# Anttwo/MACARONS

Measured on AMD Instinct MI355X. Metric: candidate-camera coverage-gain evals/sec (100k pts, 200 cams), higher is better.
Workload: dtype f32; 1 GPU; scorer: B=1 cloud x N=100000 points x C=200 cameras per GPU (BASELINE headline 100k pts / 200 cams), inputs resident in HBM; points=100000, cams_per_gpu=200, parallelism=camera-shard x1, streams=2

## Files before the change

macarons_amd/csrc/local_pct6.hip:

```cpp
#include "lp_split.h"

namespace mcr {
namespace v6 {

typedef float f32x4 __attribute__((ext_vector_type(4)));

__device__ __forceinline__ int opaque(int v) {
    asm volatile("" : "+v"(v));
    return v;
}

constexpr int PF = 3;
struct WRing { uint4 b[PF][2]; };

__device__ __forceinline__ const uint4* wptr(const float* Wp, int nt, int S, int lane) {
    return reinterpret_cast<const uint4*>(Wp) + (size_t)nt * S * 2 * 64 + lane;
}
template <int S>
__device__ __forceinline__ void wload(WRing& r, const uint4* bp) {
#pragma unroll
    for (int p = 0; p < (S < PF ? S : PF); ++p) {
        r.b[p][0] = bp[(p * 2 + 0) * 64];
        r.b[p][1] = bp[(p * 2 + 1) * 64];
    }
    __builtin_amdgcn_sched_barrier(0);
}

__device__ __forceinline__ void pin(f32x16& a, f32x16& b) { asm volatile("" : "+v"(a), "+v"(b)); }
__device__ __forceinline__ void pin(f32x16& a, f32x16& b, f32x16& c) { asm volatile("" : "+v"(a), "+v"(b), "+v"(c)); }

__device__ __forceinline__ void zero(f32x16& a) {
#pragma unroll
    for (int r = 0; r < 16; ++r) a[r] = 0.f;
}

template <int S>
__device__ __forceinline__ void gemm(f32x16 (&acc)[2], const uint4* __restrict__ A, WRing& r, const uint4* __restrict__ bp,
                                     int lane_) {
    const int lane = opaque(lane_);
    const int i = lane & 31, h = lane >> 5, key = i & 15;
    Split2 an[2];
    auto fetch = [&](int s) {
        const int c = (2 * s + h) ^ key;
#pragma unroll
        for (int mt = 0; mt < 2; ++mt) {
            an[mt].hi = A[(0 * 64 + mt * 32 + i) * 16 + c];
            an[mt].lo = A[(1 * 64 + mt * 32 + i) * 16 + c];
        }
    };
    fetch(0);
#pragma unroll
    for (int s = 0; s < S; ++s) {
        const Split2 a0 = an[0], a1 = an[1];
        if (s + 1 < S) fetch(s + 1);
        const uint4 whi = r.b[s % PF][0], wlo = r.b[s % PF][1];
        if (s + PF < S) {
            r.b[s % PF][0] = bp[((s + PF) * 2 + 0) * 64];
            r.b[s % PF][1] = bp[((s + PF) * 2 + 1) * 64];
        }
        __builtin_amdgcn_sched_barrier(0);
        acc[0] = mfma_h(wlo, a0.hi, acc[0]);
        acc[1] = mfma_h(wlo, a1.hi, acc[1]);
        acc[0] = mfma_h(whi, a0.lo, acc[0]);
        acc[1] = mfma_h(whi, a1.lo, acc[1]);
        acc[0] = mfma_h(whi, a0.hi, acc[0]);
        acc[1] = mfma_h(whi, a1.hi, acc[1]);
        pin(acc[0], acc[1]);
        __builtin_amdgcn_sched_barrier(0);
    }
}

template <int S, class Fn>
__device__ __forceinline__ void gemm_with(f32x16 (&acc)[2], const uint4* __restrict__ A, WRing& r, const uint4* __restrict__ bp,
                                          int lane_, Fn fn) {
    const int lane = opaque(lane_);
    const int i = lane & 31, h = lane >> 5, key = i & 15;
    Split2 an[2];
    auto fetch = [&](int s) {
        const int c = (2 * s + h) ^ key;
#pragma unroll
        for (int mt = 0; mt < 2; ++mt) {
            an[mt].hi = A[(0 * 64 + mt * 32 + i) * 16 + c];
            an[mt].lo = A[(1 * 64 + mt * 32 + i) * 16 + c];
        }
    };
    fetch(0);
#pragma unroll
    for (int s = 0; s < S; ++s) {
        const Split2 a0 = an[0], a1 = an[1];
        if (s + 1 < S) fetch(s + 1);
        const uint4 whi = r.b[s % PF][0], wlo = r.b[s % PF][1];
        if (s + PF < S) {
            r.b[s % PF][0] = bp[((s + PF) * 2 + 0) * 64];
            r.b[s % PF][1] = bp[((s + PF) * 2 + 1) * 64];
        }
        __builtin_amdgcn_sched_barrier(0);
        acc[0] = mfma_h(wlo, a0.hi, acc[0]);
        acc[1] = mfma_h(wlo, a1.hi, acc[1]);
        acc[0] = mfma_h(whi, a0.lo, acc[0]);
        acc[1] = mfma_h(whi, a1.lo, acc[1]);
        acc[0] = mfma_h(whi, a0.hi, acc[0]);
        acc[1] = mfma_h(whi, a1.hi, acc[1]);
        fn(s);
        pin(acc[0], acc[1]);
        __builtin_amdgcn_sched_barrier(0);
    }
}

__device__ __forceinline__ void gemm_qkv(f32x16 (&acc)[2], f32x16& acch, const uint4* __restrict__ A, WRing& r0, WRing& r1,
                                         const uint4* __restrict__ bp0, const uint4* __restrict__ bp1, int wave, int lane_) {
    constexpr int S = 8;
    const int lane = opaque(lane_);
    const int i = lane & 31, h = lane >> 5, key = i & 15, mh = wave & 1;
    Split2 an[2];
    auto fetch = [&](int s) {
        const int c = (2 * s + h) ^ key;
#pragma unroll
        for (int mt = 0; mt < 2; ++mt) {
            an[mt].hi = A[(0 * 64 + mt * 32 + i) * 16 + c];
            an[mt].lo = A[(1 * 64 + mt * 32 + i) * 16 + c];
        }
    };
    fetch(0);
#pragma unroll
    for (int s = 0; s < S; ++s) {
        const Split2 a0 = an[0], a1 = an[1];
        const Split2 ah = mh ? a1 : a0;
        if (s + 1 < S) fetch(s + 1);
        const uint4 whi = r0.b[s % PF][0], wlo = r0.b[s % PF][1], vhi = r1.b[s % PF][0], vlo = r1.b[s % PF][1];
        if (s + PF < S) {
            r0.b[s % PF][0] = bp0[((s + PF) * 2 + 0) * 64];
            r0.b[s % PF][1] = bp0[((s + PF) * 2 + 1) * 64];
            r1.b[s % PF][0] = bp1[((s + PF) * 2 + 0) * 64];
            r1.b[s % PF][1] = bp1[((s + PF) * 2 + 1) * 64];
        }
        __builtin_amdgcn_sched_barrier(0);
        acc[0] = mfma_h(wlo, a0.hi, acc[0]);
        acc[1] = mfma_h(wlo, a1.hi, acc[1]);
        acch = mfma_h(vlo, ah.hi, acch);
        acc[0] = mfma_h(whi, a0.lo, acc[0]);
        acc[1] = mfma_h(whi, a1.lo, acc[1]);
        acch = mfma_h(vhi, ah.lo, acch);
        acc[0] = mfma_h(whi, a0.hi, acc[0]);
        acc[1] = mfma_h(whi, a1.hi, acc[1]);
        acch = mfma_h(vhi, ah.hi, acch);
        pin(acc[0], acc[1], acch);
        __builtin_amdgcn_sched_barrier(0);
    }
}

__device__ __forceinline__ void scale_add_bias(f32x16& x, float scale, const float* __restrict__ vec, int nt, int lane_) {
    const float4* p = reinterpret_cast<const float4*>(vec + 32 * nt + 4 * (opaque(lane_) >> 5));
#pragma unroll
    for (int g = 0; g < 4; ++g) {
        const float4 b = p[2 * g];
        x[4 * g] = fmaf(x[4 * g], scale, b.x); x[4 * g + 1] = fmaf(x[4 * g + 1], scale, b.y);
        x[4 * g + 2] = fmaf(x[4 * g + 2], scale, b.z); x[4 * g + 3] = fmaf(x[4 * g + 3], scale, b.w);
    }
}
__device__ __forceinline__ void init_bias(f32x16& a, const float* __restrict__ vec, int nt, int lane_) {
    const float4* p = reinterpret_cast<const float4*>(vec + 32 * nt + 4 * (opaque(lane_) >> 5));
#pragma unroll
    for (int g = 0; g < 4; ++g) {
        const float4 b = p[2 * g];
        a[4 * g] = b.x; a[4 * g + 1] = b.y; a[4 * g + 2] = b.z; a[4 * g + 3] = b.w;
    }
}

__device__ __forceinline__ void put4(uint2* __restrict__ planes, int idx, float v0, float v1, float v2, float v3) {
    uint2 hi, lo;
    split2h(v0, v1, hi.x, lo.x);
    split2h(v2, v3, hi.y, lo.y);
    planes[idx] = hi;
    planes[idx + 64 * 16 * 2] = lo;
}
template <class Fn>
__device__ __forceinline__ void put_planes(uint4* __restrict__ buf, int nt, int mt, const f32x16& t, int lane_, Fn f) {
    const int lane = opaque(lane_);
    const int j = lane & 31, h = lane >> 5, key = j & 15;
    uint2* b2 = reinterpret_cast<uint2*>(buf);
    const int base = (mt * 32 + j) * 32 + h;
#pragma unroll
    for (int g = 0; g < 4; ++g) {
        put4(b2, base + (((4 * nt + g) ^ key) << 1), f(t[4 * g], g, 0), f(t[4 * g + 1], g, 1), f(t[4 * g + 2], g, 2),
             f(t[4 * g + 3], g, 3));
        __builtin_amdgcn_sched_barrier(0);
    }
}
template <class Fn>
__device__ __forceinline__ void put_quad(uint4* __restrict__ buf, int nt, int mt, int g, const f32x16& t, int row, int key, Fn f) {
    uint2* b2 = reinterpret_cast<uint2*>(buf);
    put4(b2, mt * 1024 + row + (((4 * nt + g) ^ key) << 1), f(t[4 * g]), f(t[4 * g + 1]), f(t[4 * g + 2]), f(t[4 * g + 3]));
}
template <class Fn>
__device__ __forceinline__ void put_f32(float* __restrict__ buf, int LD, int chunk0, int mt, const f32x16& t, int lane_, Fn f) {
    const int lane = opaque(lane_);
    const int j = lane & 31, h = lane >> 5, key = j & 15;
    float* row = buf + (mt * 32 + j) * LD;
#pragma unroll
    for (int g = 0; g < 4; ++g)
        *reinterpret_cast<float4*>(row + (((chunk0 + 2 * g + h) ^ key) << 2)) =
            make_float4(f(t[4 * g], g, 0), f(t[4 * g + 1], g, 1), f(t[4 * g + 2], g, 2), f(t[4 * g + 3], g, 3));
}

__device__ __forceinline__ float halves_sum(float v) {
    const unsigned c = __builtin_bit_cast(unsigned, v);
    const auto q = __builtin_amdgcn_permlane32_swap(c, c, false, false);
    return __builtin_bit_cast(float, (unsigned)q[0]) + __builtin_bit_cast(float, (unsigned)q[1]);
}
template <class Op>
__device__ __forceinline__ float rows_allreduce(float v, Op op) {
    const unsigned b = __builtin_bit_cast(unsigned, v);
    const auto r = __builtin_amdgcn_permlane16_swap(b, b, false, false);
    v = op(__builtin_bit_cast(float, (unsigned)r[0]), __builtin_bit_cast(float, (unsigned)r[1]));
    const unsigned c = __builtin_bit_cast(unsigned, v);
    const auto q = __builtin_amdgcn_permlane32_swap(c, c, false, false);
    return op(__builtin_bit_cast(float, (unsigned)q[0]), __builtin_bit_cast(float, (unsigned)q[1]));
}

__device__ __forceinline__ void ln_partial(const f32x16 (&x)[2], float2* __restrict__ St, int wave, int lane_) {
    const int lane = opaque(lane_);
#pragma unroll
    for (int mt = 0; mt < 2; ++mt) {
        float s = 0.f;
#pragma unroll
        for (int r = 0; r < 16; r += 4) s += (x[mt][r] + x[mt][r + 1]) + (x[mt][r + 2] + x[mt][r + 3]);
        const float m = halves_sum(s) * (1.0f / 32.f);
        float q = 0.f;
#pragma unroll
        for (int r = 0; r < 16; ++r) {
            const float d = x[mt][r] - m;
            q = fmaf(d, d, q);
        }
        q = halves_sum(q);
        St[wave * 64 + mt * 32 + (lane & 31)] = make_float2(m, q);
    }
}
__device__ __forceinline__ void ln_finish(const f32x16 (&x)[2], const float2* __restrict__ St, uint4* __restrict__ P, int wave,
                                          int lane_) {
    const int j = opaque(lane_) & 31;
#pragma unroll
    for (int mt = 0; mt < 2; ++mt) {
        float2 p[4];
#pragma unroll
        for (int w = 0; w < 4; ++w) p[w] = St[w * 64 + mt * 32 + j];
        const float mu = ((p[0].x + p[1].x) + (p[2].x + p[3].x)) * 0.25f;
        float m2 = (p[0].y + p[1].y) + (p[2].y + p[3].y), dd = 0.f;
#pragma unroll
        for (int w = 0; w < 4; ++w) {
            const float d = p[w].x - mu;
            dd = fmaf(d, d, dd);
        }
        m2 = fmaf(32.f, dd, m2);
        const float rstd = 1.0f / sqrtf(m2 * (1.0f / 128.f) + 1e-5f);
        put_planes(P, wave, mt, x[mt], lane_, [&](float v, int, int) { return (v - mu) * rstd; });
    }
}

#ifdef L6_TRACE
__device__ long long l6_trace_buf[64];
#define L6_T() do { if (blockIdx.x == (L6_TRACE) && tid == 0) { l6_trace_buf[tp] = clock64(); l6_trace_buf[tp ? 63 : 62] = wall_clock64(); } ++tp; } while (0)
#else
#define L6_T() do { } while (0)
#endif

__global__ __launch_bounds__(256, 2) void local_pct6_kernel(const float* __restrict__ offs, float* __restrict__ feat,
                                                          long long ld_feat, long long S,
                                                          const float* __restrict__ blob, _Float16* __restrict__ feat_h,
                                                          _Float16* __restrict__ feat_l) {
    __shared__ __attribute__((aligned(16))) uint4 P[2 * 64 * 16];
    __shared__ __attribute__((aligned(16))) uint4 H[2 * 64 * 16];
    __shared__ __attribute__((aligned(16))) float2 St[4 * 64];
    float* Pq = reinterpret_cast<float*>(P);
    float* F = reinterpret_cast<float*>(H);
    const int tid = threadIdx.x, lane0 = tid & 63;
    const int wave = __builtin_amdgcn_readfirstlane(tid >> 6);
    const float* mats = blob;
    const float* vecs = blob + L6_MATS_TOTAL;
    const float* isc = vecs + L6_SCALES;
    const long long s0 = (long long)blockIdx.x * L3_QPB;
    const int lane = lane0;
    int tp = 0; (void)tp;
    L6_T();
    WRing ring;
    f32x16 acc[2], xres[2];
    wload<1>(ring, wptr(mats + l6_mat_off(0), wave, 1, lane));
    init_bias(acc[0], vecs + L3_VEC_EMB1, wave, lane);
    init_bias(acc[1], vecs + L3_VEC_EMB1, wave, lane);
    float xyz[2][3];
    {
        const int j = lane & 31;
#pragma unroll
        for (int mt = 0; mt < 2; ++mt) {
            const int t = mt * 32 + j;
            const long long seq = s0 + (t >> 4);
            xyz[mt][0] = xyz[mt][1] = xyz[mt][2] = 0.f;
            if (seq < S) {
                const float* p = offs + (seq * 16 + (t & 15)) * 3;
                xyz[mt][0] = p[0]; xyz[mt][1] = p[1]; xyz[mt][2] = p[2];
            }
        }
        const bool lowh = lane < 32;
#pragma unroll
        for (int mt = 0; mt < 2; ++mt) {
            Split2 a;
            a.hi = make_uint4(0, 0, 0, 0); a.lo = make_uint4(0, 0, 0, 0);
            split2h(lowh ? xyz[mt][0] : 0.f, lowh ? xyz[mt][1] : 0.f, a.hi.x, a.lo.x);
            split2h(lowh ? xyz[mt][2] : 0.f, 0.f, a.hi.y, a.lo.y);
            acc[mt] = mfma_h(ring.b[0][1], a.hi, acc[mt]);
            acc[mt] = mfma_h(ring.b[0][0], a.lo, acc[mt]);
            acc[mt] = mfma_h(ring.b[0][0], a.hi, acc[mt]);
        }
    }
    L6_T();
    wload<8>(ring, wptr(mats + l6_mat_off(1), wave, 8, lane));
    {
        const float sc = isc[0];
#pragma unroll
        for (int mt = 0; mt < 2; ++mt)
            put_planes(H, wave, mt, acc[mt], lane, [&](float v, int, int) { return l3_gelu(v * sc); });
    }
    init_bias(xres[0], vecs + L3_VEC_EMB2, wave, lane);
    init_bias(xres[1], vecs + L3_VEC_EMB2, wave, lane);
    __syncthreads();
    L6_T();
    gemm<8>(xres, H, ring, wptr(mats + l6_mat_off(1), wave, 8, lane), lane);
    L6_T();
    {
        const float sc = isc[1];
#pragma unroll
        for (int mt = 0; mt < 2; ++mt)
#pragma unroll
            for (int r = 0; r < 16; ++r) xres[mt][r] *= sc;
        const bool cat = wave == 3 && lane >= 32;
#pragma unroll
        for (int mt = 0; mt < 2; ++mt) {
            xres[mt][13] = cat ? xyz[mt][0] : xres[mt][13];
            xres[mt][14] = cat ? xyz[mt][1] : xres[mt][14];
            xres[mt][15] = cat ? xyz[mt][2] : xres[mt][15];
        }
    }

#pragma unroll 1
    for (int e = 0; e < 2; ++e) {
        const float* em = mats + l6_mat_off(2) + e * (L6_MAT_QKV + 5 * L6_MAT_128);
        const float* ev = vecs + L3_VEC_ENC0 + e * L3_VEC_ENC_STRIDE;
        const float* es = isc + 2 + 6 * e;
        const float* w_out = em + L6_MAT_QKV;
        const float* w_ff1a = w_out + L6_MAT_128;
        const float* w_ff1b = w_out + L6_MAT_128 * 2;
        const float* w_ff2a = w_out + L6_MAT_128 * 3;
        const float* w_ff2b = w_out + L6_MAT_128 * 4;
        WRing ring1;
        const uint4* bq0 = wptr(em, wave, 8, lane);
        const uint4* bq1 = wptr(em, 4 + (wave >> 1), 8, lane);
        wload<8>(ring, bq0);
        wload<8>(ring1, bq1);
        L6_T();
        ln_partial(xres, St, wave, lane);
        __syncthreads();
        L6_T();
        ln_finish(xres, St, P, wave, lane);
        __syncthreads();
        L6_T();
        {
            f32x16 aq[2], ah;
            const int nth = 4 + (wave >> 1);
            init_bias(aq[0], ev, wave, lane);
            init_bias(aq[1], ev, wave, lane);
            init_bias(ah, ev, nth, lane);
            gemm_qkv(aq, ah, P, ring, ring1, bq0, bq1, wave, lane);
            L6_T();
            wload<8>(ring, wptr(w_out, wave, 8, lane));
            const float sc = es[0];
            __syncthreads();
            L6_T();
            auto fb = [&](float v, int, int) { return v * sc; };
            float* dst = wave < 2 ? Pq : F;
            const int ld = wave < 2 ? 64 : 128, c0 = wave < 2 ? 8 * wave : 8 * (wave - 2);
#pragma unroll
            for (int mt = 0; mt < 2; ++mt) put_f32(dst, ld, c0, mt, aq[mt], lane, fb);
            put_f32(F, 128, 8 * (nth - 2), wave & 1, ah, lane, fb);
        }
        __syncthreads();
        L6_T();
        {
            const int ln = opaque(lane);
            const int r0 = wave * 16, li = ln & 15, g = ln >> 4;
            const int wq = ((r0 + li) * 64) | (li << 2) | g;
            const int wv = ((r0 + 4 * g) * 128) | ((((li >> 2) | (g << 2)) << 2)) | (li & 3);
            f32x4 pr[4];
#pragma unroll
            for (int hh = 0; hh < 4; ++hh) {
                f32x4 st = {0.f, 0.f, 0.f, 0.f};
#pragma unroll
                for (int sk = 0; sk < 2; ++sk) {
                    const float kk = Pq[wq ^ ((8 + 2 * hh + sk) << 2)];
                    const float qq = Pq[wq ^ ((2 * hh + sk) << 2)];
                    st = __builtin_amdgcn_mfma_f32_16x16x4f32(kk, qq, st, 0, 0, 0);
                }
                float mx = fmaxf(fmaxf(st[0], st[1]), fmaxf(st[2], st[3]));
                mx = rows_allreduce(mx, [](float a, float b) { return fmaxf(a, b); });
                mx *= 0.35355339059327376220f;
                float den = 0.f;
#pragma unroll
                for (int r = 0; r < 4; ++r) {
                    st[r] = __expf(fmaf(st[r], 0.35355339059327376220f, -mx));
                    den += st[r];
                }
                den = rows_allreduce(den, [](float a, float b) { return a + b; });
                const float inv = __builtin_amdgcn_rcpf(den);
#pragma unroll
                for (int r = 0; r < 4; ++r) pr[hh][r] = st[r] * inv;
            }
            f32x4 o[4][2];
#pragma unroll
            for (int hh = 0; hh < 4; ++hh)
#pragma unroll
                for (int nt = 0; nt < 2; ++nt) {
                    o[hh][nt] = f32x4{0.f, 0.f, 0.f, 0.f};
#pragma unroll
                    for (int sk = 0; sk < 4; ++sk) {
                        const float vv = F[sk * 128 + (wv ^ (((hh * 8 + nt * 4) ^ sk) << 2))];
                        o[hh][nt] = __builtin_amdgcn_mfma_f32_16x16x4f32(vv, pr[hh][sk], o[hh][nt], 0, 0, 0);
                    }
                }
            asm volatile("s_waitcnt lgkmcnt(0)" ::: "memory");
            uint2* p2 = reinterpret_cast<uint2*>(P);
            const int base = (r0 + li) * 32 + (g & 1);
#pragma unroll
            for (int hh = 0; hh < 4; ++hh)
#pragma unroll
                for (int nt = 0; nt < 2; ++nt)
                    put4(p2, base + (((4 * hh + 2 * nt + (g >> 1)) ^ li) << 1), o[hh][nt][0], o[hh][nt][1], o[hh][nt][2], o[hh][nt][3]);
        }
        L6_T();
        scale_add_bias(xres[0], es[16 + 1], ev + 192, wave, lane);
        scale_add_bias(xres[1], es[16 + 1], ev + 192, wave, lane);
        __syncthreads();
        L6_T();
        gemm<8>(xres, P, ring, wptr(w_out, wave, 8, lane), lane);
        L6_T();
        wload<8>(ring, wptr(w_ff1a, wave, 8, lane));
        {
            const float sc = es[1];
#pragma unroll
            for (int mt = 0; mt < 2; ++mt)
#pragma unroll
                for (int r = 0; r < 16; ++r) xres[mt][r] *= sc;
        }
        ln_partial(xres, St, wave, lane);
        init_bias(acc[0], ev + 192 + 128, wave, lane);
        init_bias(acc[1], ev + 192 + 128, wave, lane);
        __syncthreads();
        L6_T();
        ln_finish(xres, St, P, wave, lane);
        __syncthreads();
        L6_T();
        gemm<8>(acc, P, ring, wptr(w_ff1a, wave, 8, lane), lane);
        L6_T();
        wload<8>(ring, wptr(w_ff1b, wave, 8, lane));
        f32x16 accb[2];
        init_bias(accb[0], ev + 192 + 128 + 128, wave, lane);
        init_bias(accb[1], ev + 192 + 128 + 128, wave, lane);
        const int pq_lane = opaque(lane), pq_row = (pq_lane & 31) * 32 + (pq_lane >> 5), pq_key = pq_lane & 15;
        {
            const float sc = es[2];
            gemm_with<8>(accb, P, ring, wptr(w_ff1b, wave, 8, lane), lane, [&](int s_) {
                put_quad(H, wave, s_ >> 2, s_ & 3, acc[s_ >> 2], pq_row, pq_key, [&](float v) { return l3_gelu(v * sc); });
            });
        }
        L6_T();
        wload<8>(ring, wptr(w_ff2a, wave, 8, lane));
        scale_add_bias(xres[0], es[16 + 4], ev + 192 + 128 + 256, wave, lane);
        scale_add_bias(xres[1], es[16 + 4], ev + 192 + 128 + 256, wave, lane);
        __syncthreads();
        L6_T();
        {
            const float sc = es[3];
            gemm_with<8>(xres, H, ring, wptr(w_ff2a, wave, 8, lane), lane, [&](int s_) {
                put_quad(P, wave, s_ >> 2, s_ & 3, accb[s_ >> 2], pq_row, pq_key, [&](float v) { return l3_gelu(v * sc); });
            });
        }
        L6_T();
        wload<8>(ring, wptr(w_ff2b, wave, 8, lane));
        __syncthreads();
        L6_T();
        L6_T();
        gemm<8>(xres, P, ring, wptr(w_ff2b, wave, 8, lane), lane);
        L6_T();
        {
            const float sc = es[4];
#pragma unroll
            for (int mt = 0; mt < 2; ++mt)
#pragma unroll
                for (int r = 0; r < 16; ++r) xres[mt][r] *= sc;
        }
    }
    L6_T();
    wload<8>(ring, wptr(mats + l6_mat_off(14), wave, 8, lane));
    ln_partial(xres, St, wave, lane);
    init_bias(acc[0], vecs + L3_VEC_LIN0, wave, lane);
    init_bias(acc[1], vecs + L3_VEC_LIN0, wave, lane);
    __syncthreads();
    ln_finish(xres, St, P, wave, lane);
    __syncthreads();
    gemm<8>(acc, P, ring, wptr(mats + l6_mat_off(14), wave, 8, lane), lane);
    {
        const float sc = isc[14];
#pragma unroll
        for (int mt = 0; mt < 2; ++mt)
            put_f32(F, 128, 8 * wave, mt, acc[mt], lane, [&](float v, int, int) { return v * sc; });
    }
    __syncthreads();
    L6_T();
#pragma unroll
    for (int r = 0; r < 2; ++r) {
        const int o = tid + r * 256, q = o >> 7, c = o & 127;
        if (s0 + q < S) {
            float mx = -__builtin_inff(), sm = 0.f;
#pragma unroll
            for (int j = 0; j < 16; ++j) {
                const int row = q * 16 + j;
                const float v = F[row * 128 + ((((c >> 2) ^ (row & 15)) << 2) | (c & 3))];
                mx = fmaxf(mx, v);
                sm += v;
            }
            const float av = sm * (1.0f / 16.f);
            if (feat_h) {
                unsigned hi, lo;
                split2h(mx, av, hi, lo);
                const long long o2 = (s0 + q) * ld_feat + c;
                feat_h[o2] = __builtin_bit_cast(_Float16, (unsigned short)(hi & 0xffffu));
                feat_h[o2 + 128] = __builtin_bit_cast(_Float16, (unsigned short)(hi >> 16));
                feat_l[o2] = __builtin_bit_cast(_Float16, (unsigned short)(lo & 0xffffu));
                feat_l[o2 + 128] = __builtin_bit_cast(_Float16, (unsigned short)(lo >> 16));
            } else {
                feat[(s0 + q) * ld_feat + c] = mx;
                feat[(s0 + q) * ld_feat + 128 + c] = av;
            }
        }
    }
    L6_T();
}

}

#ifdef L6_TRACE
extern "C" int mcr_dev_read_trace(long long* out) { return (int)hipMemcpyFromSymbol(out, HIP_SYMBOL(v6::l6_trace_buf), sizeof(long long) * 64); }
#endif

void launch_local_pct6(hipStream_t s, const float* offs, float* feat, int64_t ld_feat, int64_t S, const float* blob, void* feat_h,
                       void* feat_l) {
    if (S <= 0) return;
    hipLaunchKernelGGL(v6::local_pct6_kernel, dim3((unsigned)cdiv(S, L3_QPB)), dim3(256), 0, s, offs, feat, (long long)ld_feat,
                       (long long)S, blob, (_Float16*)feat_h, (_Float16*)feat_l);
}

int local_pct6_blob_floats() { return L6_BLOB_FLOATS; }

}
```

Before: 5.056 million evals/s.

## Run local attention QK and PV with split-f16 MFMA instead of f32 MFMA

Q/K/V are now written into LDS in the hi/lo f16 plane layout, not as plain f32. QK^T is computed with a single 16x16x32 f16 MFMA per head, replacing two 16x16x4 f32 MFMAs. PV uses split-half probabilities with two f16 MFMAs, and V is read through ds_read_tr16 transposed LDS loads. The aim is to cut MFMA count and LDS read traffic in the attention block, at the cost of some precision: it depends on how put_planes packs the hi/lo planes, and only one plane of Q/K appears to be used.

```diff
diff --git a/macarons_amd/csrc/local_pct6.hip b/macarons_amd/csrc/local_pct6.hip
--- a/macarons_amd/csrc/local_pct6.hip
+++ b/macarons_amd/csrc/local_pct6.hip
@@ -271,7 +271,6 @@
     __shared__ __attribute__((aligned(16))) uint4 P[2 * 64 * 16];
     __shared__ __attribute__((aligned(16))) uint4 H[2 * 64 * 16];
     __shared__ __attribute__((aligned(16))) float2 St[4 * 64];
-    float* Pq = reinterpret_cast<float*>(P);
     float* F = reinterpret_cast<float*>(H);
     const int tid = threadIdx.x, lane0 = tid & 63;
     const int wave = __builtin_amdgcn_readfirstlane(tid >> 6);
@@ -376,29 +375,31 @@
             __syncthreads();
             L6_T();
             auto fb = [&](float v, int, int) { return v * sc; };
-            float* dst = wave < 2 ? Pq : F;
-            const int ld = wave < 2 ? 64 : 128, c0 = wave < 2 ? 8 * wave : 8 * (wave - 2);
-#pragma unroll
-            for (int mt = 0; mt < 2; ++mt) put_f32(dst, ld, c0, mt, aq[mt], lane, fb);
-            put_f32(F, 128, 8 * (nth - 2), wave & 1, ah, lane, fb);
+            uint4* dst = wave < 2 ? P : H;
+            const int ntd = wave < 2 ? wave : wave - 2;
+#pragma unroll
+            for (int mt = 0; mt < 2; ++mt) put_planes(dst, ntd, mt, aq[mt], lane, fb);
+            put_planes(H, nth - 2, wave & 1, ah, lane, fb);
         }
         __syncthreads();
         L6_T();
         {
+            typedef _Float16 h16x8 __attribute__((ext_vector_type(8)));
+            typedef short s16x4 __attribute__((ext_vector_type(4)));
+            typedef __attribute__((address_space(3))) s16x4 lds_s16x4;
             const int ln = opaque(lane);
             const int r0 = wave * 16, li = ln & 15, g = ln >> 4;
-            const int wq = ((r0 + li) * 64) | (li << 2) | g;
-            const int wv = ((r0 + 4 * g) * 128) | ((((li >> 2) | (g << 2)) << 2)) | (li & 3);
-            f32x4 pr[4];
+            const int wk = (((g >> 1) * 64 + r0 + li) * 16) | li;
+            const int wq = (((g & 1) * 64 + r0 + li) * 16) | li;
+            const int vrow = 4 * g + (li >> 2);
+            const int wv = ((((r0 + vrow) * 16) | (vrow ^ ((li & 3) >> 1))) << 4) | ((li & 1) << 3);
+            uint4 ph[4], pl[4];
 #pragma unroll
             for (int hh = 0; hh < 4; ++hh) {
-                f32x4 st = {0.f, 0.f, 0.f, 0.f};
-#pragma unroll
-                for (int sk = 0; sk < 2; ++sk) {
-                    const float kk = Pq[wq ^ ((8 + 2 * hh + sk) << 2)];
-                    const float qq = Pq[wq ^ ((2 * hh + sk) << 2)];
-                    st = __builtin_amdgcn_mfma_f32_16x16x4f32(kk, qq, st, 0, 0, 0);
-                }
+                const uint4 kf = P[wk ^ (4 + hh)];
+                const uint4 qf = P[wq ^ hh];
+                f32x4 st = __builtin_amdgcn_mfma_f32_16x16x32_f16(__builtin_bit_cast(h16x8, kf), __builtin_bit_cast(h16x8, qf),
+                                                                  f32x4{0.f, 0.f, 0.f, 0.f}, 0, 0, 0);
                 float mx = fmaxf(fmaxf(st[0], st[1]), fmaxf(st[2], st[3]));
                 mx = rows_allreduce(mx, [](float a, float b) { return fmaxf(a, b); });
                 mx *= 0.35355339059327376220f;
@@ -410,20 +411,24 @@
                 }
                 den = rows_allreduce(den, [](float a, float b) { return a + b; });
                 const float inv = __builtin_amdgcn_rcpf(den);
-#pragma unroll
-                for (int r = 0; r < 4; ++r) pr[hh][r] = st[r] * inv;
+                uint2 hi, lo;
+                split2h(st[0] * inv, st[1] * inv, hi.x, lo.x);
+                split2h(st[2] * inv, st[3] * inv, hi.y, lo.y);
+                ph[hh] = make_uint4(hi.x, hi.y, hi.x, hi.y);
+                pl[hh] = make_uint4(lo.x, lo.y, lo.x, lo.y);
             }
             f32x4 o[4][2];
+            const char* Hb = reinterpret_cast<const char*>(H);
 #pragma unroll
             for (int hh = 0; hh < 4; ++hh)
 #pragma unroll
                 for (int nt = 0; nt < 2; ++nt) {
-                    o[hh][nt] = f32x4{0.f, 0.f, 0.f, 0.f};
-#pragma unroll
-                    for (int sk = 0; sk < 4; ++sk) {
-                        const float vv = F[sk * 128 + (wv ^ (((hh * 8 + nt * 4) ^ sk) << 2))];
-                        o[hh][nt] = __builtin_amdgcn_mfma_f32_16x16x4f32(vv, pr[hh][sk], o[hh][nt], 0, 0, 0);
-                    }
+                    const char* va = Hb + (wv ^ ((2 * hh + nt) << 5));
+                    const s16x4 vh = __builtin_amdgcn_ds_read_tr16_b64_v4i16((lds_s16x4*)va);
+                    const s16x4 vl = __builtin_amdgcn_ds_read_tr16_b64_v4i16((lds_s16x4*)(va + 64 * 16 * 16));
+                    const h16x8 vf = __builtin_bit_cast(h16x8, __builtin_shufflevector(vh, vl, 0, 1, 2, 3, 4, 5, 6, 7));
+                    o[hh][nt] = __builtin_amdgcn_mfma_f32_16x16x32_f16(vf, __builtin_bit_cast(h16x8, pl[hh]), f32x4{0.f, 0.f, 0.f, 0.f}, 0, 0, 0);
+                    o[hh][nt] = __builtin_amdgcn_mfma_f32_16x16x32_f16(vf, __builtin_bit_cast(h16x8, ph[hh]), o[hh][nt], 0, 0, 0);
                 }
             asm volatile("s_waitcnt lgkmcnt(0)" ::: "memory");
             uint2* p2 = reinterpret_cast<uint2*>(P);
```

Result: no change. 5.039 million evals/s (median of 3 runs) (-0.3%).
